# sohmandal/classpose

Measured on AMD Instinct MI355X. Metric: wsi_tiles_per_sec, higher is better.
Workload: dtype bf16; 1 GPU; configs[1]: synthetic 10000x10000 WSI (1936 tiles), tile 256 / overlap 32, conic 7 classes, ViT-L ClassTransformer depth 24 random-init, batch 32 sub-tiles = 8 WSI tiles/step, every step a distinct batch of the rank's shard (tiles sharded k % n_gpus, at most 256 distinct batches resident, longer runs wrap) streamed pinned host -> hipMemcpyAsync inside the timed region (the reader decodes ahead int; slide=10000, tile=256, overlap=32, batch_subtiles=32, distinct_batches=145, records_gathered=2048, decode_ahead_batches_at_t0=4, device_resident_batches_at_t0=1

## Files before the change

classpose_amd/_lib.py:

```python
from __future__ import annotations

import ctypes as C
import os
import subprocess

_HERE = os.path.dirname(os.path.abspath(__file__))
LIB_PATH = os.path.join(_HERE, "libclasspose_hip.so")
DEBUG_LIB_PATH = os.path.join(_HERE, "libclasspose_hip_debug.so")
CSRC = os.path.join(_HERE, "csrc")

ABI_VERSION = 3
DT_BF16, DT_F16, DT_F32 = 0, 1, 2
DTYPE_CODE = {"bf16": DT_BF16, "fp16": DT_F16, "fp32": DT_F32}
PROF_KINDS = ("fc1", "attention", "qkv", "proj", "fc2", "patch_embed", "neck_head")
FC1_KERNEL_NAME = "k_gemm4w<GELU + folded LayerNorm, one wave per SIMD> = void k_gemm4w<1, 0, false>(Gemm4wArgs)"


class CpxTiling(C.Structure):
    _fields_ = [("H", C.c_int), ("W", C.c_int), ("ypad1", C.c_int), ("xpad1", C.c_int),
                ("Ly", C.c_int), ("Lx", C.c_int), ("ny", C.c_int), ("nx", C.c_int),
                ("bsize", C.c_int), ("augment", C.c_int),
                ("ystart", C.c_int * 16), ("xstart", C.c_int * 16)]


# ... 115 lines not shown
    "cpx_head_wgrad_slab_rows": (_i, []),
    "cpx_head_wgrad_workspace_bytes": (_sz, [_i, _i]),
    "cpx_head_wgrad": (_i, [_p, _p, _i, _i, _i, _p, _p, _p, _sz, _p]),
    "cpx_adamw_step": (_i, [_p, _p, _p, _p, C.c_longlong, _d, _d, _d, _d, _d, _d, _d, _p]),
    "cpx_find_contours_ccomp_host": (_i, [_p, _i, _i, _p, _i, _p, _p, _p, _i]),
    "cpx_polygonize_workspace_bytes": (_sz, [_i, _i, _i, _i]),
    "cpx_polygonize_device": (_i, [_p, _p, _p, _i, _i, _i, _i, _d, _p, _p, _i, _p, _p, _p, _p]),
    "cpx_polygonize_host": (_i, [_p, _i, _i, _p, _i, _d, _d, _d, _p, _i, _p]),
    "cpx_dedup_pairs_workspace_bytes": (_sz, [_i, _i, _i]),
    "cpx_dedup_pairs": (_i, [_p, _i, _d, _d, _d, _i, _i, _d, _p, C.c_longlong, _p, _p, _sz, _p]),
    "cpx_write_geojson": (_i, [C.c_char_p, C.c_char_p, _p, C.c_int64, _p, _p, _p, _p, C.c_int64, _p, _i, _d, _d, _i]),
}
_PRIVATE = {
    "cpx_gemm_set_variant": (None, [_i]),
    "cpx_attention_set_variant": (None, [_i]),
    "cpx_gemm_set_nt": (None, [_i]),
    "cpx_follow_set_early_exit": (None, [_i]),
    "cpx_follow_set_lds_window": (None, [_i]),
    "cpx_gemm_set_reverse": (None, [_i]),
    "cpx_attention_set_xcd_order": (None, [_i]),
    "cpx_gemm_set_big": (None, [_i]),
    "cpx_gemm_set_persistent": (None, [_i]),
    "cpx_gemm_set_persistent_qkv": (None, [_i]),
    "cpx_postproc_set_fused": (None, [_i]),
    "cpx_gemm_set_direct": (None, [_i]),
    "cpx_gemm4w": (_i, [_p, _p, _i, _i, _i, _p, _p, _i, _p]),
    "cpx_gemm4w_set_variant": (None, [_i]),
    "cpx_gemm_set_4w": (None, [_i]),
    "cpx_net_set_mlp_parts": (None, [_i]),
    "cpx_gemm_set_balanced": (None, [_i]),
# ... 115 lines not shown
```

classpose_amd/csrc/cpx_attn2w.hip:

```cpp
#include "cpx_internal.h"
#include <type_traits>

namespace {
typedef __attribute__((ext_vector_type(8))) __bf16 bf16x8;
typedef __attribute__((ext_vector_type(8))) _Float16 f16x8;
typedef __attribute__((ext_vector_type(16))) float f32x16;
typedef __attribute__((ext_vector_type(2))) float f32x2;
typedef __attribute__((ext_vector_type(2))) __bf16 bf16x2;
typedef __attribute__((ext_vector_type(2))) _Float16 f16x2;
typedef __attribute__((ext_vector_type(4))) unsigned u32x4;

template <bool F16>
__device__ __forceinline__ f32x16 mfma32(const u32x4 &a, const u32x4 &b, f32x16 c) {
    if constexpr (F16)
        return __builtin_amdgcn_mfma_f32_32x32x16_f16(__builtin_bit_cast(f16x8, a), __builtin_bit_cast(f16x8, b), c, 0, 0, 0);
    else
        return __builtin_amdgcn_mfma_f32_32x32x16_bf16(__builtin_bit_cast(bf16x8, a), __builtin_bit_cast(bf16x8, b), c, 0, 0, 0);
}
template <bool F16>
__device__ __forceinline__ unsigned pack2(float lo, float hi) {
    f32x2 v = {lo, hi};
    if constexpr (F16) return __builtin_bit_cast(unsigned, __builtin_convertvector(v, f16x2));
    else return __builtin_bit_cast(unsigned, __builtin_convertvector(v, bf16x2));
}
__device__ __forceinline__ int pi_perm(int r) { return (r & ~12) | ((r & 4) << 1) | ((r & 8) >> 1); }
template <int OFF>
__device__ __forceinline__ u32x4 a2w_read128(unsigned addr) {
    u32x4 v;
    asm volatile("ds_read_b128 %0, %1 offset:%2" : "=v"(v) : "v"(addr), "n"(OFF));
    return v;
}
}

#define A2W_THREADS 256
#define A2W_SLOT 8192
#define A2W_G_LD 66
#define A2W_LDS_BYTES (4 * A2W_SLOT + 8 * 32 * A2W_G_LD * 2)
static_assert(A2W_LDS_BYTES <= 80 * 1024, "two workgroups per CU");

template <bool F16>
__global__ void __launch_bounds__(A2W_THREADS, 2) k_attention2w(const unsigned short *__restrict__ qkv,
                                                                 const unsigned short *__restrict__ vT,
                                                                 const unsigned short *__restrict__ relh,
                                                                 const unsigned short *__restrict__ relw,
                                                                 unsigned short *__restrict__ out, int xcd_order) {
    extern __shared__ __attribute__((aligned(16))) char a2w_smem[];
    const int tid = threadIdx.x, lane = tid & 63;
    const int wave = __builtin_amdgcn_readfirstlane(tid >> 6);
    const int r = lane & 31, h2 = lane >> 5;
    const int lin = (blockIdx.z * gridDim.y + blockIdx.y) * gridDim.x + blockIdx.x;
    int rg = blockIdx.x, head = blockIdx.y, s = blockIdx.z;
    if (xcd_order) {
        const int j = lin >> 3, pair = (j >> 2) * 8 + (lin & 7);
        rg = j & 3; head = pair & 15; s = pair >> 4;
    }
    const int qh0 = rg * 8 + wave * 2;
    const size_t tok0 = (size_t)s * 1024;
    const int kkey = tid >> 3, vd = tid >> 2;
    const unsigned short *ksrc = qkv + (tok0 + kkey) * 3072 + 1024 + head * 64 + (((tid & 7) ^ ((kkey >> 1) & 7)) * 8);
    const unsigned short *vsrc = vT + (((size_t)s * 16 + head) * 64 + vd) * 1024 + (((tid & 3) ^ ((vd >> 2) & 3)) * 8);
    char *dma_dst = a2w_smem + wave * 1024;
    auto issue = [&](int kh) {
        char *d = dma_dst + (kh & 3) * A2W_SLOT;
        __builtin_amdgcn_global_load_lds((const __attribute__((address_space(1))) void *)(ksrc + (size_t)kh * 32 * 3072),
                                         (__attribute__((address_space(3))) void *)d, 16, 0, 0);
        __builtin_amdgcn_global_load_lds((const __attribute__((address_space(1))) void *)(vsrc + kh * 32),
                                         (__attribute__((address_space(3))) void *)(d + 4096), 16, 0, 0);
    };
    issue(0); issue(1); issue(2);

    u32x4 qf[2][4];
#pragma unroll
    for (int c = 0; c < 2; ++c) {
        const unsigned short *qrow = qkv + (tok0 + (qh0 + c) * 32 + r) * 3072 + head * 64;
#pragma unroll
        for (int ks = 0; ks < 4; ++ks) qf[c][ks] = *reinterpret_cast<const u32x4 *>(qrow + 16 * ks + 8 * h2);
    }
    f32x16 GW[2];
#pragma unroll
    for (int c = 0; c < 2; ++c) {
        _Float16 *G = reinterpret_cast<_Float16 *>(a2w_smem + 4 * A2W_SLOT) + (wave * 2 + c) * 32 * A2W_G_LD;
        auto compute_G = [&](const unsigned short *table) {
// ... 19 lines not shown
    asm volatile("s_waitcnt vmcnt(0) lgkmcnt(0)" ::: "memory");
    __builtin_amdgcn_s_barrier();

    const unsigned lds0 = (unsigned)(size_t)(__attribute__((address_space(3))) char *)a2w_smem;
    const int krow = pi_perm(r);
    unsigned ka[4], va[4];
#pragma unroll
    for (int ks = 0; ks < 4; ++ks) ka[ks] = lds0 + (unsigned)(krow * 128 + (((2 * ks + h2) ^ ((krow >> 1) & 7)) * 16));
#pragma unroll
    for (int db = 0; db < 2; ++db)
#pragma unroll
        for (int st = 0; st < 2; ++st) {
            const int d = db * 32 + r;
            va[db * 2 + st] = lds0 + 4096u + (unsigned)(d * 64 + (((2 * st + h2) ^ ((d >> 2) & 3)) * 16));
        }
    unsigned gaddr[2];
#pragma unroll
    for (int c = 0; c < 2; ++c)
        gaddr[c] = lds0 + 4u * A2W_SLOT + (unsigned)((((wave * 2 + c) * 32 + r) * A2W_G_LD + qh0 + c + 31) * 2);

    u32x4 kf[4], vf[4];
    unsigned ghb[2];
    kf[0] = a2w_read128<0>(ka[0]); kf[1] = a2w_read128<0>(ka[1]);
    kf[2] = a2w_read128<0>(ka[2]); kf[3] = a2w_read128<0>(ka[3]);
    asm volatile("ds_read_u16 %0, %1" : "=v"(ghb[0]) : "v"(gaddr[0]));
    asm volatile("ds_read_u16 %0, %1" : "=v"(ghb[1]) : "v"(gaddr[1]));
    asm volatile("s_waitcnt lgkmcnt(0)" : "+v"(kf[0]), "+v"(kf[1]), "+v"(kf[2]), "+v"(kf[3]), "+v"(ghb[0]), "+v"(ghb[1])::"memory");
    f32x16 S[2], O0[2], O1[2];
    S[0] = mfma32<F16>(kf[0], qf[0][0], GW[0]);
    S[0] = mfma32<F16>(kf[1], qf[0][1], S[0]);
// ... 73 lines not shown
        if constexpr (TAIL == 0) issue(kh + 3);
        unsigned ghn[2] = {0u, 0u};
        if constexpr (TAIL < 3) {
            asm volatile("ds_read_u16 %0, %1" : "=v"(ghn[0]) : "v"(gaddr[0] - 2u * (unsigned)(kh + 1)));
            asm volatile("ds_read_u16 %0, %1" : "=v"(ghn[1]) : "v"(gaddr[1] - 2u * (unsigned)(kh + 1)));
        }
        __builtin_amdgcn_sched_barrier(0);
        qk(C1{});
        if constexpr (!FIRST) pv(C1{});
        softmax(C0{}, ghb[0]);
        __builtin_amdgcn_sched_barrier(0);
        if constexpr (TAIL < 3) {
            kf[0] = a2w_read128<SN * A2W_SLOT>(ka[0]); kf[1] = a2w_read128<SN * A2W_SLOT>(ka[1]);
            kf[2] = a2w_read128<SN * A2W_SLOT>(ka[2]); kf[3] = a2w_read128<SN * A2W_SLOT>(ka[3]);
        }
        vf[0] = a2w_read128<SL * A2W_SLOT>(va[0]); vf[1] = a2w_read128<SL * A2W_SLOT>(va[1]);
        vf[2] = a2w_read128<SL * A2W_SLOT>(va[2]); vf[3] = a2w_read128<SL * A2W_SLOT>(va[3]);
        asm volatile("s_waitcnt lgkmcnt(0)" : "+v"(kf[0]), "+v"(kf[1]), "+v"(kf[2]), "+v"(kf[3]), "+v"(vf[0]), "+v"(vf[1]),
                     "+v"(vf[2]), "+v"(vf[3]), "+v"(ghn[0]), "+v"(ghn[1])::"memory");
        __builtin_amdgcn_sched_barrier(0);
        if constexpr (TAIL < 3) qk(C0{});
        pv(C0{});
        softmax(C1{}, ghb[1]);
        __builtin_amdgcn_sched_barrier(0);
        ghb[0] = ghn[0]; ghb[1] = ghn[1];
    };
    using T0 = integral_constant<int, 0>;
    using NF = std::false_type;
    tile(0, integral_constant<int, 0>{}, integral_constant<int, 1>{}, T0{}, std::true_type{});
    tile(1, integral_constant<int, 1>{}, integral_constant<int, 2>{}, T0{}, NF{});
    tile(2, integral_constant<int, 2>{}, integral_constant<int, 3>{}, T0{}, NF{});
    tile(3, integral_constant<int, 3>{}, integral_constant<int, 0>{}, T0{}, NF{});
// ... 16 lines not shown
        unsigned short *orow = out + (tok0 + (qh0 + c) * 32 + r) * 1024 + head * 64;
#pragma unroll
        for (int db = 0; db < 2; ++db)
#pragma unroll
            for (int g4 = 0; g4 < 4; g4 += 2) {
                const f32x16 &O = db ? O1[c] : O0[c];
                unsigned ax = pack2<F16>(O[4 * g4 + 0] * inv, O[4 * g4 + 1] * inv), ay = pack2<F16>(O[4 * g4 + 2] * inv, O[4 * g4 + 3] * inv);
                unsigned bx = pack2<F16>(O[4 * g4 + 4] * inv, O[4 * g4 + 5] * inv), by = pack2<F16>(O[4 * g4 + 6] * inv, O[4 * g4 + 7] * inv);
                const auto rx = __builtin_amdgcn_permlane32_swap(ax, bx, false, false);
                const auto ry = __builtin_amdgcn_permlane32_swap(ay, by, false, false);
                *reinterpret_cast<uint4 *>(orow + db * 32 + 8 * g4 + 8 * h2) = make_uint4(rx[0], ry[0], rx[1], ry[1]);
            }
    }
}

int cpx_attention2w_launch(int dtype, const void *qkv, const void *vT, const void *rel_h, const void *rel_w,
                           int n_subtiles, void *out, int xcd_order, hipStream_t s) {
    static CpxOncePerDevice once;
    once([] {
        (void)hipFuncSetAttribute((const void *)k_attention2w<true>, hipFuncAttributeMaxDynamicSharedMemorySize, A2W_LDS_BYTES);
        (void)hipFuncSetAttribute((const void *)k_attention2w<false>, hipFuncAttributeMaxDynamicSharedMemorySize, A2W_LDS_BYTES);
    });
    const dim3 grid(4, 16, n_subtiles);
    if (dtype == CPX_DT_F16)
        hipLaunchKernelGGL((k_attention2w<true>), grid, dim3(A2W_THREADS), A2W_LDS_BYTES, s, (const unsigned short *)qkv,
                           (const unsigned short *)vT, (const unsigned short *)rel_h, (const unsigned short *)rel_w,
                           (unsigned short *)out, xcd_order);
    else
        hipLaunchKernelGGL((k_attention2w<false>), grid, dim3(A2W_THREADS), A2W_LDS_BYTES, s, (const unsigned short *)qkv,
                           (const unsigned short *)vT, (const unsigned short *)rel_h, (const unsigned short *)rel_w,
                           (unsigned short *)out, xcd_order);
    CPX_CHECK_LAUNCH();
    return CPX_OK;
}
```

classpose_amd/csrc/cpx_gemm.hip:

```cpp
#include "cpx_internal.h"
#include <type_traits>

typedef __attribute__((ext_vector_type(8))) __bf16 bf16x8;
typedef __attribute__((ext_vector_type(8))) _Float16 f16x8;
typedef __attribute__((ext_vector_type(4))) float f32x4;

#define BM 128
#define BN 128
#define BK 64
#define GEMM_THREADS 256
#define TILE_BYTES (128 * 128)
#define STAGE_BYTES (2 * TILE_BYTES)

template <bool NT_POSSIBLE, bool WT_POSSIBLE = false>
__device__ __forceinline__ void st16(void *p, uint4 v, bool nt, bool wt = false) {
    if (WT_POSSIBLE && wt) {
        typedef unsigned u32x4_t __attribute__((ext_vector_type(4)));
        u32x4_t w = {v.x, v.y, v.z, v.w};
        if (NT_POSSIBLE && nt) asm volatile("global_store_dwordx4 %0, %1, off sc1 nt" ::"v"(p), "v"(w) : "memory");
        else asm volatile("global_store_dwordx4 %0, %1, off sc1" ::"v"(p), "v"(w) : "memory");
    } else if (NT_POSSIBLE && nt) {
        typedef unsigned u32x4_t __attribute__((ext_vector_type(4)));
        u32x4_t w = {v.x, v.y, v.z, v.w};
        __builtin_nontemporal_store(w, reinterpret_cast<u32x4_t *>(p));
// ... 979 lines not shown
                    const int mlh = it * 16 + (tid >> 5);
                    uint4 vv = *reinterpret_cast<const uint4 *>(stg + mlh * G2_EPI_LD + c16 * 16);
                    const int ml = hm * 128 + mlh;
                    const size_t go = (size_t)(m0 + ml) * g.ld_out + n0 + c16 * 8;
                    if constexpr (EPI == CPX_EPI_RESID_BF16) {
                        const uint4 rr = rres[it];
                        unsigned a[4] = {vv.x, vv.y, vv.z, vv.w}, b[4] = {rr.x, rr.y, rr.z, rr.w};
#pragma unroll
                        for (int i = 0; i < 4; ++i) {
                            float lo = from_half<F16>(a[i] & 0xFFFF) + from_half<F16>(b[i] & 0xFFFF);
                            float hi = from_half<F16>(a[i] >> 16) + from_half<F16>(b[i] >> 16);
                            a[i] = pack2<F16>(lo, hi);
                        }
                        vv = make_uint4(a[0], a[1], a[2], a[3]);
                    }
                    if (!DBG || !(g.dbg & 1) || vv.x == 0x12345678u) st16<EPI == CPX_EPI_QKV_BF16, EPI == CPX_EPI_RESID_BF16 || EPI == CPX_EPI_QKV_BF16>((unsigned short *)g.out + go, vv, (g.nt_out & (n0 < 1024 ? 1 : 2)) != 0,
                                                                                        (g.nt_out & (EPI == CPX_EPI_QKV_BF16 ? 16 : 8)) != 0);
                    if constexpr (STATS) {
                        unsigned a[4] = {vv.x, vv.y, vv.z, vv.w};
                        float sm = 0.f, sq = 0.f;
#pragma unroll
                        for (int i = 0; i < 4; ++i) {
                            const float lo = from_half<F16>(a[i] & 0xFFFF), hi = from_half<F16>(a[i] >> 16);
                            sm += lo + hi; sq += lo * lo + hi * hi;
                        }
                        sm = half_wave_sum(sm); sq = half_wave_sum(sq);
                        if (c16 == 16)
                            *reinterpret_cast<float2 *>(g.stats_out + ((size_t)(m0 + ml) * LN_SLOTS + tile_n) * 2) = make_float2(sm, sq);
                    }
                }
                asm volatile("s_waitcnt lgkmcnt(0)" ::: "memory");
                G2_BAR();
// ... 95 lines not shown
                        }
                    }
                    if (f1) launch_gemm256_flags<EPI, F16, F1 | G2F_DBG>(a, s);
                    else launch_gemm256_flags<EPI, F16, G2F_DBG>(a, s);
                    return true;
                }
            }
#endif
            if constexpr (EPI == CPX_EPI_GELU_BF16) {
                if (g_gemm_4w && f1 && a.bias && a.K >= 256 && (a.K / 64) % 2 == 0 &&
                    cpx_gemm4w_gelu_ln(F16 ? 1 : 0, a.A, a.W, a.M, a.N, a.K, a.bias, a.ln_stats, a.ln_colsum, a.out, a.ld_out, s))
                    return true;
            }
            constexpr bool DIRECT_OK = EPI == CPX_EPI_GELU_BF16
#ifdef CPX_DEBUG
                                       || (EPI != CPX_EPI_RESID_BF16 && EPI != CPX_EPI_QKV_BF16)
#endif
                ;
            constexpr bool BAL_OK = EPI == CPX_EPI_RESID_BF16 && !F16;
            const bool bal = BAL_OK && g_gemm_bal != 0 && f1 && a.K >= 256;
            if constexpr (DIRECT_OK) {
                if ((EPI == CPX_EPI_GELU_BF16 ? g_gemm_direct != 0 : g_gemm_direct == 2) && (size_t)a.M * (size_t)a.ld_out * 2 < ((size_t)1 << 31)) {
                    if (f1) launch_gemm256_flags<EPI, F16, F1 | G2F_DIRECT>(a, s);
                    else launch_gemm256_flags<EPI, F16, G2F_DIRECT>(a, s);
                    return true;
                }
            }
            if constexpr (BAL_OK) {
                if (bal) {
                    launch_gemm256_flags<EPI, F16, F1 | G2F_BAL>(a, s);
                    return true;
// ... 56 lines not shown
    if (epilogue == CPX_EPI_F32) return 0;
    if (!g_gemm_big || M % 256 || N % 256 || K < 128) return 0;
    if ((K / 64) % 2 && epilogue != CPX_EPI_POS_BF16) return 0;
    return (M / 256) * (N / 256) >= 256;
}

int cpx_gemm_half(int dtype, const void *A, const void *Wt, int M, int N, int K, int epilogue,
                  const float *bias, const void *aux, void *out, int ld_out,
                  const float *ln_stats, const float *ln_colsum, float *stats_out, void *stream) {
    CPX_REQUIRE(A && Wt && out && (dtype == CPX_DT_BF16 || dtype == CPX_DT_F16));
    const bool f16 = dtype == CPX_DT_F16;
    CPX_REQUIRE(M > 0 && N > 0 && K > 0 && M % BM == 0 && N % BN == 0 && K % BK == 0);
    CPX_REQUIRE(ld_out >= N && ld_out % 4 == 0);
    CPX_REQUIRE((epilogue != CPX_EPI_RESID_BF16 && epilogue != CPX_EPI_POS_BF16 && epilogue != CPX_EPI_QKV_BF16) || aux);
    CPX_REQUIRE(epilogue != CPX_EPI_QKV_BF16 || (N == 3072 && M % 1024 == 0));
    CPX_REQUIRE(!ln_stats || (ln_colsum && epilogue != CPX_EPI_RESID_BF16));
    CPX_REQUIRE(!stats_out || ((epilogue == CPX_EPI_RESID_BF16 || epilogue == CPX_EPI_POS_BF16) && N == 1024 && cpx_gemm_half_uses_big_tile(M, N, K, epilogue)));
    GemmArgs a;
    a.A = (const unsigned short *)A; a.W = (const unsigned short *)Wt;
    a.M = M; a.N = N; a.K = K; a.bias = bias; a.aux = aux; a.out = out; a.ld_out = ld_out;
    a.tiles_n = N / BN; a.n_blocks = (M / BM) * (N / BN);
    a.ln_stats = ln_stats; a.ln_colsum = ln_colsum; a.stats_out = stats_out; a.l2_block = g_gemm_l2; a.dbg = g_gemm_dbg; a.nt_out = g_gemm_nt;
    a.rev_m = (g_gemm_rev && K >= 4096) ? 1 : 0;
    a.conv_c = 0;
    hipStream_t s = (hipStream_t)stream;
    switch (epilogue) {
        case CPX_EPI_BF16: launch_gemm<CPX_EPI_BF16>(a, s, f16); break;
        case CPX_EPI_GELU_BF16: launch_gemm<CPX_EPI_GELU_BF16>(a, s, f16); break;
        case CPX_EPI_RESID_BF16: launch_gemm<CPX_EPI_RESID_BF16>(a, s, f16); break;
        case CPX_EPI_F32: launch_gemm<CPX_EPI_F32>(a, s, f16); break;
        case CPX_EPI_POS_BF16: launch_gemm<CPX_EPI_POS_BF16>(a, s, f16); break;
        case CPX_EPI_RELU_BF16: launch_gemm<CPX_EPI_RELU_BF16>(a, s, f16); break;
        case CPX_EPI_QKV_BF16: launch_gemm<CPX_EPI_QKV_BF16>(a, s, f16); break;
        default: CPX_REQUIRE(!"unknown epilogue");
    }
    CPX_CHECK_LAUNCH();
    return CPX_OK;
}

int cpx_conv3_half(int dtype, const void *x, const void *Wt, int M, int N, int C, int epilogue, const float *bias,
                   void *out, int ld_out, void *stream) {
    CPX_REQUIRE(x && Wt && out && (dtype == CPX_DT_BF16 || dtype == CPX_DT_F16));
    CPX_REQUIRE(M > 0 && M % 1024 == 0 && N > 0 && N % BN == 0 && C > 0 && C % BK == 0);
    CPX_REQUIRE(ld_out >= N && ld_out % 4 == 0 && (epilogue == CPX_EPI_BF16 || epilogue == CPX_EPI_RELU_BF16));
    GemmArgs a;
    a.A = (const unsigned short *)x; a.W = (const unsigned short *)Wt;
    a.M = M; a.N = N; a.K = 9 * C; a.bias = bias; a.aux = nullptr; a.out = out; a.ld_out = ld_out;
    a.tiles_n = N / BN; a.n_blocks = (M / BM) * (N / BN);
// ... 51 lines not shown
```

classpose_amd/csrc/cpx_internal.h:

```cpp
#pragma once
#include "cpx_common.h"
#include <atomic>

struct CpxOncePerDevice {
    std::atomic<unsigned long long> done{0};
    template <class F>
    void operator()(F &&f) {
        int dev = 0;
        (void)hipGetDevice(&dev);
        const unsigned long long bit = 1ull << (dev & 63);
        if (!(done.load(std::memory_order_acquire) & bit)) {
            f();
            done.fetch_or(bit, std::memory_order_release);
        }
    }
};

enum { CPX_PROF_FC1 = 0, CPX_PROF_ATTN = 1, CPX_PROF_QKV = 2, CPX_PROF_PROJ = 3, CPX_PROF_FC2 = 4,
       CPX_PROF_PE = 5,
       CPX_PROF_TAIL = 6,
       CPX_PROF_KINDS = 7 };
struct CpxProf {
    hipEvent_t *ev = nullptr;
    int *kind = nullptr;
// ... 11 lines not shown
    (void)hipEventRecord(p->ev[2 * p->n + 1], s);
    ++p->n;
}

int cpx_gemm_half(int dtype, const void *A, const void *Wt, int M, int N, int K, int epilogue, const float *bias,
                  const void *aux, void *out, int ld_out, const float *ln_stats, const float *ln_colsum,
                  float *stats_out, void *stream);
int cpx_conv3_half(int dtype, const void *x, const void *Wt, int M, int N, int C, int epilogue, const float *bias,
                   void *out, int ld_out, void *stream);
int cpx_row_stats_half(int dtype, const void *x, int rows, float *stats, void *stream);
int cpx_gemm_half_uses_big_tile(int M, int N, int K, int epilogue);
int cpx_gemm4w_gelu_ln(int f16, const void *A, const void *W, int M, int N, int K, const float *bias, const float *ln_stats, const float *ln_colsum,
                       void *out, int ld_out, hipStream_t s);
int cpx_layernorm_half(int dtype, const void *x, const float *w, const float *b, int rows, int C, float eps,
                       void *out, void *stream);
int cpx_attention_half(int dtype, const void *qkv, const void *rel_h, const void *rel_w, int n_subtiles, void *vT_ws,
                       void *out, void *stream, bool transpose_v);
int cpx_attention2w_launch(int dtype, const void *qkv, const void *vT, const void *rel_h, const void *rel_w,
                           int n_subtiles, void *out, int xcd_order, hipStream_t s);

int cpx_gemm_f32(const float *A, const float *Wt, int M, int N, int K, int epilogue, const float *bias,
                 const float *aux, float *out, int ld_out, void *stream);
int cpx_layernorm_f32(const float *x, const float *w, const float *b, int rows, int C, float eps, float *out,
                      void *stream);
int cpx_attention_f32(const float *qkv, const float *rel_h, const float *rel_w, int n_subtiles, float *out,
                      void *stream);
size_t cpx_net_f32_workspace_bytes(int n_subtiles);
size_t cpx_net_f32_neck_offset(int n_subtiles);
int cpx_net_forward_f32(const cpx_net_weights *w, const void *patches, int nS, float *head, void *workspace,
                        size_t workspace_bytes, void *stream);

int cpx_unet_head_run(int dtype, const cpx_conv_op *ops, int n_ops, const void *feat, int nS, float *head, int ld_head,
                      int col0, void *workspace, size_t ws_bytes, void *stream);
size_t cpx_unet_ws_bytes(int dtype, const cpx_conv_op *ops, int n_ops, int nS);
// ... 1 lines not shown
```

classpose_amd/csrc/cpx_net.hip:

```cpp
#include "cpx_internal.h"
#include <algorithm>

typedef __attribute__((ext_vector_type(8))) __bf16 bf16x8;
typedef __attribute__((ext_vector_type(8))) _Float16 f16x8;
typedef __attribute__((ext_vector_type(16))) float f32x16;

template <bool F16>
__device__ __forceinline__ f32x16 mfma32(const uint4 &a, const uint4 &b, f32x16 c) {
    if constexpr (F16)
        return __builtin_amdgcn_mfma_f32_32x32x16_f16(*reinterpret_cast<const f16x8 *>(&a),
                                                      *reinterpret_cast<const f16x8 *>(&b), c, 0, 0, 0);
    else
        return __builtin_amdgcn_mfma_f32_32x32x16_bf16(*reinterpret_cast<const bf16x8 *>(&a),
                                                       *reinterpret_cast<const bf16x8 *>(&b), c, 0, 0, 0);
}
template <bool F16>
__device__ __forceinline__ unsigned short h_from_f32(float f) {
    if constexpr (F16) { _Float16 h = (_Float16)f; return *reinterpret_cast<unsigned short *>(&h); }
    else return f32_to_bf16(f);
}
template <bool F16>
__device__ __forceinline__ float f32_from_h(unsigned short u) {
    if constexpr (F16) return (float)*reinterpret_cast<_Float16 *>(&u);
    else return bf16_to_f32(u);
// ... 293 lines not shown
#pragma unroll
    for (int db = 0; db < 2; ++db)
#pragma unroll
        for (int g4 = 0; g4 < 4; g4 += 2) {
            const f32x16 &O = db ? O1 : O0;
            unsigned ax = pack2<F16>(O[4 * g4 + 0] * inv, O[4 * g4 + 1] * inv), ay = pack2<F16>(O[4 * g4 + 2] * inv, O[4 * g4 + 3] * inv);
            unsigned bx = pack2<F16>(O[4 * g4 + 4] * inv, O[4 * g4 + 5] * inv), by = pack2<F16>(O[4 * g4 + 6] * inv, O[4 * g4 + 7] * inv);
            const auto rx = __builtin_amdgcn_permlane32_swap(ax, bx, false, false);
            const auto ry = __builtin_amdgcn_permlane32_swap(ay, by, false, false);
            *reinterpret_cast<uint4 *>(orow + db * 32 + 8 * g4 + 8 * h2) = make_uint4(rx[0], ry[0], rx[1], ry[1]);
        }
}

CPX_SWITCH(g_att_xcd, 1);
CPX_SWITCH(g_att_v8, 2);
#ifdef CPX_DEBUG
extern "C" void cpx_attention_set_variant(int v8) { g_att_v8 = v8; }
extern "C" void cpx_attention_set_xcd_order(int v) { g_att_xcd = v; }
#endif
extern "C" int cpx_attention_relpos(const void *qkv, const void *rel_h, const void *rel_w,
                                    int n_subtiles, void *vT_ws, void *out, void *stream) {
    return cpx_attention_half(CPX_DT_BF16, qkv, rel_h, rel_w, n_subtiles, vT_ws, out, stream, true);
}
extern "C" int cpx_attention(int dtype, const void *qkv, const void *rel_h, const void *rel_w,
                             int n_subtiles, void *vT_ws, void *out, void *stream) {
    if (dtype == CPX_DT_F32)
        return cpx_attention_f32((const float *)qkv, (const float *)rel_h, (const float *)rel_w, n_subtiles, (float *)out, stream);
    return cpx_attention_half(dtype, qkv, rel_h, rel_w, n_subtiles, vT_ws, out, stream, true);
}
int cpx_attention_half(int dtype, const void *qkv, const void *rel_h, const void *rel_w, int n_subtiles,
                       void *vT_ws, void *out, void *stream, bool transpose_v) {
    CPX_REQUIRE(qkv && rel_h && rel_w && vT_ws && out && n_subtiles > 0);
    CPX_REQUIRE(dtype == CPX_DT_BF16 || dtype == CPX_DT_F16);
#ifdef CPX_DEBUG
    CPX_REQUIRE(g_att_v8 == 2 || g_att_v8 == 7);
#endif
    hipStream_t s = (hipStream_t)stream;
    if (transpose_v)
        hipLaunchKernelGGL(k_v_transpose, dim3(16, 16, n_subtiles), dim3(256), 0, s,
                           (const unsigned short *)qkv, (unsigned short *)vT_ws);
#ifdef CPX_DEBUG
    if (g_att_v8 == 7) {
        const dim3 grid4(8, 16, n_subtiles);
        static CpxOncePerDevice once4;
        once4([] {
            (void)hipFuncSetAttribute((const void *)k_attention4p<true>, hipFuncAttributeMaxDynamicSharedMemorySize, A4_LDS_BYTES);
            (void)hipFuncSetAttribute((const void *)k_attention4p<false>, hipFuncAttributeMaxDynamicSharedMemorySize, A4_LDS_BYTES);
        });
        if (dtype == CPX_DT_F16)
            hipLaunchKernelGGL((k_attention4p<true>), grid4, dim3(ATT_THREADS), A4_LDS_BYTES, s, (const unsigned short *)qkv, (const unsigned short *)vT_ws,
                               (const unsigned short *)rel_h, (const unsigned short *)rel_w, (unsigned short *)out, g_att_xcd);
        else
            hipLaunchKernelGGL((k_attention4p<false>), grid4, dim3(ATT_THREADS), A4_LDS_BYTES, s, (const unsigned short *)qkv, (const unsigned short *)vT_ws,
                               (const unsigned short *)rel_h, (const unsigned short *)rel_w, (unsigned short *)out, g_att_xcd);
        CPX_CHECK_LAUNCH();
        return CPX_OK;
    }
#endif
    return cpx_attention2w_launch(dtype, qkv, vT_ws, rel_h, rel_w, n_subtiles, out, g_att_xcd, s);
}

struct NetWs {
    size_t off_x, off_xn, off_qkv, off_vt, off_ao, off_h, off_neck, off_neck2, off_st, total;
};
static NetWs net_ws(int nS) {
    NetWs w; size_t o = 0; const size_t M = (size_t)nS * 1024;
    auto take = [&](size_t b) { size_t r = o; o = cpx_align_up(o + b, 256); return r; };
    w.off_x = take(M * 1024 * 2);
    w.off_xn = take(M * 1024 * 2);
    w.off_qkv = take(M * 3072 * 2);
    w.off_vt = take(M * 1024 * 2);
    w.off_ao = take(M * 1024 * 2);
    w.off_h = take(M * 4096 * 2);
    w.off_neck = take(M * 256 * 2);
    w.off_neck2 = take(M * 256 * 2);
    w.off_st = take(M * 8 * sizeof(float));
    w.total = o;
    return w;
}
extern "C" size_t cpx_net_workspace_bytes(int n_subtiles, int dtype) {
    if (n_subtiles <= 0) return 0;
    return dtype == CPX_DT_F32 ? cpx_net_f32_workspace_bytes(n_subtiles) : net_ws(n_subtiles).total;
}

extern "C" size_t cpx_net_neck_offset(int n_subtiles, int dtype) {
    if (n_subtiles <= 0 || dtype < CPX_DT_BF16 || dtype > CPX_DT_F32) return 0;
// ... 60 lines not shown
    row0 = pt * 16384;
    rows = pt + 1 < parts ? 16384 : n_subtiles * 1024 - row0;
}

extern "C" int cpx_net_forward(const cpx_net_weights *w, const void *patches, int nS, float *head,
                               void *workspace, size_t workspace_bytes, void *stream) {
    CPX_REQUIRE(w && patches && head && workspace && nS > 0);
    CPX_REQUIRE(w->depth > 0 && w->blocks && w->ld_head % 128 == 0 && w->ld_head >= w->n_head_cols);
    CPX_REQUIRE(w->dtype == CPX_DT_BF16 || w->dtype == CPX_DT_F16 || w->dtype == CPX_DT_F32);
    if (w->dtype == CPX_DT_F32) return cpx_net_forward_f32(w, patches, nS, head, workspace, workspace_bytes, stream);
    NetWs L = net_ws(nS);
    CPX_REQUIRE(workspace_bytes >= L.total);
    const int dt = w->dtype;
    char *ws = (char *)workspace;
    const int M = nS * 1024;
    void *x = ws + L.off_x, *xn = ws + L.off_xn, *qkv = ws + L.off_qkv, *vt = ws + L.off_vt,
         *ao = ws + L.off_ao, *hb = ws + L.off_h, *nk = ws + L.off_neck, *nk2 = ws + L.off_neck2;
    CpxProf *prof = (CpxProf *)w->prof;
    if (prof) prof->phase = (prof->phase + 1) % prof->stride;
    hipStream_t hs = (hipStream_t)stream;
    int rc;
#define RUN(call) do { rc = (call); if (rc) return rc; } while (0)
#define GEMM(A_, W_, N_, K_, EPI_, B_, AUX_, OUT_, LD_) \
    cpx_gemm_half(dt, A_, W_, M, N_, K_, EPI_, B_, AUX_, OUT_, LD_, nullptr, nullptr, nullptr, stream)
#define TIMED(kind_, layer_, call_) do { const bool t_ = cpx_prof_begin(prof, kind_, layer_, hs); RUN(call_); if (t_) cpx_prof_end(prof, hs); } while (0)
    float *st = (float *)(ws + L.off_st);
    const bool fuse = w->fuse_ln != 0;
    const bool big_stats = fuse && cpx_gemm_half_uses_big_tile(M, 1024, 1024, CPX_EPI_RESID_BF16) &&
                           cpx_gemm_half_uses_big_tile(M, 1024, 4096, CPX_EPI_RESID_BF16);
    const bool pe_stats = big_stats && cpx_gemm_half_uses_big_tile(M, 1024, 192, CPX_EPI_POS_BF16);
    TIMED(CPX_PROF_PE, 0, cpx_gemm_half(dt, patches, w->pe_w, M, 1024, 192, CPX_EPI_POS_BF16, w->pe_b, w->pos, x, 1024, nullptr, nullptr,
                                        pe_stats ? st : nullptr, stream));
    if (fuse && !pe_stats) RUN(cpx_row_stats_half(dt, x, M, st, stream));
    for (int i = 0; i < w->depth; ++i) {
        const cpx_block_weights &b = w->blocks[i];
        if (fuse) {
            TIMED(CPX_PROF_QKV, i, cpx_gemm_half(dt, x, b.qkv_w, M, 3072, 1024, CPX_EPI_QKV_BF16, b.qkv_b, vt, qkv, 3072, st, b.qkv_colsum, nullptr, stream));
            TIMED(CPX_PROF_ATTN, i, cpx_attention_half(dt, qkv, b.rel_h, b.rel_w, nS, vt, ao, stream, false));
            TIMED(CPX_PROF_PROJ, i, cpx_gemm_half(dt, ao, b.proj_w, M, 1024, 1024, CPX_EPI_RESID_BF16, b.proj_b, x, x, 1024, nullptr, nullptr, big_stats ? st : nullptr, stream));
            if (!big_stats) RUN(cpx_row_stats_half(dt, x, M, st, stream));
            const int parts = big_stats ? cpx_net_mlp_parts(nS, dt) : 1;
            for (int pt = 0; pt < parts; ++pt) {
                int r0, Mp;
                mlp_part_rows(nS, parts, pt, r0, Mp);
                char *xp = (char *)x + (size_t)r0 * 1024 * 2;
                float *stp = st + (size_t)r0 * 8;
                TIMED(CPX_PROF_FC1, i, cpx_gemm_half(dt, xp, b.fc1_w, Mp, 4096, 1024, CPX_EPI_GELU_BF16, b.fc1_b, nullptr, hb, 4096, stp, b.fc1_colsum, nullptr, stream));
                TIMED(CPX_PROF_FC2, i, cpx_gemm_half(dt, hb, b.fc2_w, Mp, 1024, 4096, CPX_EPI_RESID_BF16, b.fc2_b, xp, xp, 1024, nullptr, nullptr, big_stats ? stp : nullptr, stream));
            }
            if (!big_stats) RUN(cpx_row_stats_half(dt, x, M, st, stream));
            continue;
        }
        RUN(cpx_layernorm_half(dt, x, b.ln1_w, b.ln1_b, M, 1024, 1e-6f, xn, stream));
        TIMED(CPX_PROF_QKV, i, GEMM(xn, b.qkv_w, 3072, 1024, CPX_EPI_QKV_BF16, b.qkv_b, vt, qkv, 3072));
        TIMED(CPX_PROF_ATTN, i, cpx_attention_half(dt, qkv, b.rel_h, b.rel_w, nS, vt, ao, stream, false));
        TIMED(CPX_PROF_PROJ, i, GEMM(ao, b.proj_w, 1024, 1024, CPX_EPI_RESID_BF16, b.proj_b, x, x, 1024));
        RUN(cpx_layernorm_half(dt, x, b.ln2_w, b.ln2_b, M, 1024, 1e-6f, xn, stream));
        TIMED(CPX_PROF_FC1, i, GEMM(xn, b.fc1_w, 4096, 1024, CPX_EPI_GELU_BF16, b.fc1_b, nullptr, hb, 4096));
        TIMED(CPX_PROF_FC2, i, GEMM(hb, b.fc2_w, 1024, 4096, CPX_EPI_RESID_BF16, b.fc2_b, x, x, 1024));
    }
    const bool t_tail = cpx_prof_begin(prof, CPX_PROF_TAIL, 0, hs);
    RUN(GEMM(x, w->neck0_w, 256, 1024, CPX_EPI_BF16, nullptr, nullptr, nk, 256));
    RUN(cpx_layernorm_half(dt, nk, w->neck_ln1_w, w->neck_ln1_b, M, 256, 1e-6f, nk2, stream));
    RUN(cpx_conv3_half(dt, nk2, w->neck2_w, M, 256, 256, CPX_EPI_BF16, nullptr, nk, 256, stream));
    RUN(cpx_layernorm_half(dt, nk, w->neck_ln2_w, w->neck_ln2_b, M, 256, 1e-6f, nk2, stream));
    RUN(GEMM(nk2, w->head_w, w->ld_head, 256, CPX_EPI_F32, w->head_b, nullptr, head, w->ld_head));
    if (w->n_unet_ops > 0) {
        const size_t need = cpx_unet_ws_bytes(dt, w->unet_ops, w->n_unet_ops, nS);
        CPX_REQUIRE(workspace_bytes >= L.total + need);
// ... 189 lines not shown
```

include/classpose_hip_debug.h:

```cpp
#ifndef CLASSPOSE_HIP_DEBUG_H
#define CLASSPOSE_HIP_DEBUG_H
#ifdef __cplusplus
extern "C" {
#endif
void cpx_gemm_set_variant(int glds);
void cpx_gemm_set_big(int on);
void cpx_gemm_set_persistent(int on);
void cpx_gemm_set_persistent_qkv(int on);
void cpx_gemm_set_l2_block(int on);
void cpx_gemm_set_reverse(int on);
void cpx_gemm_set_direct(int mode);
void cpx_gemm_set_balanced(int on);
int cpx_gemm4w(const void *A, const void *W, int M, int N, int K, const float *bias, void *out, int ld_out, void *stream);
void cpx_gemm_set_4w(int on);
void cpx_gemm4w_set_variant(int v);
void cpx_gemm_set_dbg(int mask);
void cpx_net_set_mlp_parts(int on);
void cpx_attention_set_xcd_order(int on);
void cpx_attention_set_variant(int v);
void cpx_postproc_set_fused(int on);
void cpx_gemm_set_nt(int on);
void cpx_follow_set_early_exit(int on);
void cpx_follow_set_lds_window(int on);
int cpx_row_stats_dt(int dtype, const void *x, int rows, float *stats, void *stream);
int cpx_gemm_ln_dt(int dtype, const void *A, const void *Wt, int M, int N, int K, int epilogue,
                   const float *bias, const void *aux, void *out, int ld_out,
                   const float *ln_stats, const float *ln_colsum, float *stats_out, void *stream);
int cpx_im2col3_f32_debug(const float *x, int n_subtiles, float *out, void *stream);
struct cpx_conv_op;
int cpx_unet_head_layout(const struct cpx_conv_op *ops, int n_ops, int n_subtiles, int dtype, size_t *dst_off, int *ld);
#ifdef __cplusplus
}
#endif
#endif
// ... 1 lines not shown
```

Before: 383.6 tiles/s.

## Read V rows directly in attention via LDS transpose reads, drop V transpose output

New measurement: 385.3 tiles/s, median of 6. No clear change (+0.4%).

```diff
diff --git a/classpose_amd/_lib.py b/classpose_amd/_lib.py
--- a/classpose_amd/_lib.py
+++ b/classpose_amd/_lib.py
@@ -153,6 +153,7 @@
 _PRIVATE = {
     "cpx_gemm_set_variant": (None, [_i]),
     "cpx_attention_set_variant": (None, [_i]),
+    "cpx_attention_set_v_rows": (None, [_i]),
     "cpx_gemm_set_nt": (None, [_i]),
     "cpx_follow_set_early_exit": (None, [_i]),
     "cpx_follow_set_lds_window": (None, [_i]),
diff --git a/classpose_amd/csrc/cpx_attn2w.hip b/classpose_amd/csrc/cpx_attn2w.hip
--- a/classpose_amd/csrc/cpx_attn2w.hip
+++ b/classpose_amd/csrc/cpx_attn2w.hip
@@ -9,6 +9,7 @@
 typedef __attribute__((ext_vector_type(2))) __bf16 bf16x2;
 typedef __attribute__((ext_vector_type(2))) _Float16 f16x2;
 typedef __attribute__((ext_vector_type(4))) unsigned u32x4;
+typedef __attribute__((ext_vector_type(2))) unsigned u32x2;
 
 template <bool F16>
 __device__ __forceinline__ f32x16 mfma32(const u32x4 &a, const u32x4 &b, f32x16 c) {
@@ -30,6 +31,13 @@
     asm volatile("ds_read_b128 %0, %1 offset:%2" : "=v"(v) : "v"(addr), "n"(OFF));
     return v;
 }
+template <int OFF>
+__device__ __forceinline__ u32x4 a2w_read_tr(unsigned addr) {
+    u32x2 lo, hi;
+    asm volatile("ds_read_b64_tr_b16 %0, %1 offset:%2" : "=v"(lo) : "v"(addr), "n"(OFF));
+    asm volatile("ds_read_b64_tr_b16 %0, %1 offset:%2" : "=v"(hi) : "v"(addr), "n"(OFF + 512));
+    return (u32x4){lo[0], lo[1], hi[0], hi[1]};
+}
 }
 
 #define A2W_THREADS 256
@@ -38,7 +46,7 @@
 #define A2W_LDS_BYTES (4 * A2W_SLOT + 8 * 32 * A2W_G_LD * 2)
 static_assert(A2W_LDS_BYTES <= 80 * 1024, "two workgroups per CU");
 
-template <bool F16>
+template <bool F16, bool VT>
 __global__ void __launch_bounds__(A2W_THREADS, 2) k_attention2w(const unsigned short *__restrict__ qkv,
                                                                  const unsigned short *__restrict__ vT,
                                                                  const unsigned short *__restrict__ relh,
@@ -59,13 +67,23 @@
     const int kkey = tid >> 3, vd = tid >> 2;
     const unsigned short *ksrc = qkv + (tok0 + kkey) * 3072 + 1024 + head * 64 + (((tid & 7) ^ ((kkey >> 1) & 7)) * 8);
     const unsigned short *vsrc = vT + (((size_t)s * 16 + head) * 64 + vd) * 1024 + (((tid & 3) ^ ((vd >> 2) & 3)) * 8);
+    const unsigned kvoff = (unsigned)(kkey * 3072 + (((tid & 7) ^ ((kkey >> 1) & 7)) * 8)) * 2u;
+    const unsigned vvoff = (unsigned)(kkey * 3072 + (((tid & 7) ^ (((kkey >> 1) & 1) << 2)) * 8)) * 2u;
+    const __amdgpu_buffer_rsrc_t rsrc = __builtin_amdgcn_make_buffer_rsrc((void *)(qkv + tok0 * 3072), 0, 1024 * 3072 * 2, 0x00020000);
+    const unsigned ksoff = (unsigned)(1024 + head * 64) * 2u;
     char *dma_dst = a2w_smem + wave * 1024;
     auto issue = [&](int kh) {
         char *d = dma_dst + (kh & 3) * A2W_SLOT;
-        __builtin_amdgcn_global_load_lds((const __attribute__((address_space(1))) void *)(ksrc + (size_t)kh * 32 * 3072),
-                                         (__attribute__((address_space(3))) void *)d, 16, 0, 0);
-        __builtin_amdgcn_global_load_lds((const __attribute__((address_space(1))) void *)(vsrc + kh * 32),
-                                         (__attribute__((address_space(3))) void *)(d + 4096), 16, 0, 0);
+        if constexpr (VT) {
+            __builtin_amdgcn_global_load_lds((const __attribute__((address_space(1))) void *)(ksrc + (size_t)kh * 32 * 3072),
+                                             (__attribute__((address_space(3))) void *)d, 16, 0, 0);
+            __builtin_amdgcn_global_load_lds((const __attribute__((address_space(1))) void *)(vsrc + kh * 32),
+                                             (__attribute__((address_space(3))) void *)(d + 4096), 16, 0, 0);
+        } else {
+            const unsigned so = ksoff + (unsigned)kh * (32u * 3072u * 2u);
+            __builtin_amdgcn_raw_ptr_buffer_load_lds(rsrc, (__attribute__((address_space(3))) void *)d, 16, kvoff, so, 0, 0);
+            __builtin_amdgcn_raw_ptr_buffer_load_lds(rsrc, (__attribute__((address_space(3))) void *)(d + 4096), 16, vvoff, so + 2048u, 0, 0);
+        }
     };
     issue(0); issue(1); issue(2);
 
@@ -115,6 +133,13 @@
             const int d = db * 32 + r;
             va[db * 2 + st] = lds0 + 4096u + (unsigned)(d * 64 + (((2 * st + h2) ^ ((d >> 2) & 3)) * 16));
         }
+    unsigned vb[2];
+    {
+        const int gi = lane & 15, g1 = (lane >> 4) & 1, q = gi >> 2, p = gi & 3;
+#pragma unroll
+        for (int db = 0; db < 2; ++db)
+            vb[db] = lds0 + 4096u + (unsigned)((8 * h2 + q) * 128 + 16 * ((4 * db + 2 * g1 + (p >> 1)) ^ (((q >> 1) & 1) << 2)) + 8 * (p & 1));
+    }
     unsigned gaddr[2];
 #pragma unroll
     for (int c = 0; c < 2; ++c)
@@ -218,8 +243,13 @@
             kf[0] = a2w_read128<SN * A2W_SLOT>(ka[0]); kf[1] = a2w_read128<SN * A2W_SLOT>(ka[1]);
             kf[2] = a2w_read128<SN * A2W_SLOT>(ka[2]); kf[3] = a2w_read128<SN * A2W_SLOT>(ka[3]);
         }
-        vf[0] = a2w_read128<SL * A2W_SLOT>(va[0]); vf[1] = a2w_read128<SL * A2W_SLOT>(va[1]);
-        vf[2] = a2w_read128<SL * A2W_SLOT>(va[2]); vf[3] = a2w_read128<SL * A2W_SLOT>(va[3]);
+        if constexpr (VT) {
+            vf[0] = a2w_read128<SL * A2W_SLOT>(va[0]); vf[1] = a2w_read128<SL * A2W_SLOT>(va[1]);
+            vf[2] = a2w_read128<SL * A2W_SLOT>(va[2]); vf[3] = a2w_read128<SL * A2W_SLOT>(va[3]);
+        } else {
+            vf[0] = a2w_read_tr<SL * A2W_SLOT>(vb[0]); vf[1] = a2w_read_tr<SL * A2W_SLOT + 2048>(vb[0]);
+            vf[2] = a2w_read_tr<SL * A2W_SLOT>(vb[1]); vf[3] = a2w_read_tr<SL * A2W_SLOT + 2048>(vb[1]);
+        }
         asm volatile("s_waitcnt lgkmcnt(0)" : "+v"(kf[0]), "+v"(kf[1]), "+v"(kf[2]), "+v"(kf[3]), "+v"(vf[0]), "+v"(vf[1]),
                      "+v"(vf[2]), "+v"(vf[3]), "+v"(ghn[0]), "+v"(ghn[1])::"memory");
         __builtin_amdgcn_sched_barrier(0);
@@ -266,22 +296,33 @@
     }
 }
 
-int cpx_attention2w_launch(int dtype, const void *qkv, const void *vT, const void *rel_h, const void *rel_w,
-                           int n_subtiles, void *out, int xcd_order, hipStream_t s) {
+template <bool VT>
+static int attention2w_launch(int dtype, const void *qkv, const void *vT, const void *rel_h, const void *rel_w,
+                              int n_subtiles, void *out, int xcd_order, hipStream_t s) {
     static CpxOncePerDevice once;
     once([] {
-        (void)hipFuncSetAttribute((const void *)k_attention2w<true>, hipFuncAttributeMaxDynamicSharedMemorySize, A2W_LDS_BYTES);
-        (void)hipFuncSetAttribute((const void *)k_attention2w<false>, hipFuncAttributeMaxDynamicSharedMemorySize, A2W_LDS_BYTES);
+        (void)hipFuncSetAttribute((const void *)k_attention2w<true, VT>, hipFuncAttributeMaxDynamicSharedMemorySize, A2W_LDS_BYTES);
+        (void)hipFuncSetAttribute((const void *)k_attention2w<false, VT>, hipFuncAttributeMaxDynamicSharedMemorySize, A2W_LDS_BYTES);
     });
     const dim3 grid(4, 16, n_subtiles);
     if (dtype == CPX_DT_F16)
-        hipLaunchKernelGGL((k_attention2w<true>), grid, dim3(A2W_THREADS), A2W_LDS_BYTES, s, (const unsigned short *)qkv,
+        hipLaunchKernelGGL((k_attention2w<true, VT>), grid, dim3(A2W_THREADS), A2W_LDS_BYTES, s, (const unsigned short *)qkv,
                            (const unsigned short *)vT, (const unsigned short *)rel_h, (const unsigned short *)rel_w,
                            (unsigned short *)out, xcd_order);
     else
-        hipLaunchKernelGGL((k_attention2w<false>), grid, dim3(A2W_THREADS), A2W_LDS_BYTES, s, (const unsigned short *)qkv,
+        hipLaunchKernelGGL((k_attention2w<false, VT>), grid, dim3(A2W_THREADS), A2W_LDS_BYTES, s, (const unsigned short *)qkv,
                            (const unsigned short *)vT, (const unsigned short *)rel_h, (const unsigned short *)rel_w,
                            (unsigned short *)out, xcd_order);
     CPX_CHECK_LAUNCH();
     return CPX_OK;
 }
+int cpx_attention2w_launch(int dtype, const void *qkv, const void *rel_h, const void *rel_w, int n_subtiles, void *out,
+                           int xcd_order, hipStream_t s) {
+    return attention2w_launch<false>(dtype, qkv, nullptr, rel_h, rel_w, n_subtiles, out, xcd_order, s);
+}
+#ifdef CPX_DEBUG
+int cpx_attention2w_vt_launch(int dtype, const void *qkv, const void *vT, const void *rel_h, const void *rel_w,
+                              int n_subtiles, void *out, int xcd_order, hipStream_t s) {
+    return attention2w_launch<true>(dtype, qkv, vT, rel_h, rel_w, n_subtiles, out, xcd_order, s);
+}
+#endif
diff --git a/classpose_amd/csrc/cpx_gemm.hip b/classpose_amd/csrc/cpx_gemm.hip
--- a/classpose_amd/csrc/cpx_gemm.hip
+++ b/classpose_amd/csrc/cpx_gemm.hip
@@ -1017,8 +1017,9 @@
                         }
                         vv = make_uint4(a[0], a[1], a[2], a[3]);
                     }
-                    if (!DBG || !(g.dbg & 1) || vv.x == 0x12345678u) st16<EPI == CPX_EPI_QKV_BF16, EPI == CPX_EPI_RESID_BF16 || EPI == CPX_EPI_QKV_BF16>((unsigned short *)g.out + go, vv, (g.nt_out & (n0 < 1024 ? 1 : 2)) != 0,
-                                                                                        (g.nt_out & (EPI == CPX_EPI_QKV_BF16 ? 16 : 8)) != 0);
+                    constexpr bool QKV = EPI == CPX_EPI_QKV_BF16 || EPI == CPX_EPI_QKV_ROWS;
+                    if (!DBG || !(g.dbg & 1) || vv.x == 0x12345678u) st16<QKV, EPI == CPX_EPI_RESID_BF16 || QKV>((unsigned short *)g.out + go, vv, (g.nt_out & (n0 < 1024 ? 1 : n0 < 2048 ? 2 : 4)) != 0,
+                                                                                        (g.nt_out & (QKV ? 16 : 8)) != 0);
                     if constexpr (STATS) {
                         unsigned a[4] = {vv.x, vv.y, vv.z, vv.w};
                         float sm = 0.f, sq = 0.f;
@@ -1144,7 +1145,7 @@
             }
             constexpr bool DIRECT_OK = EPI == CPX_EPI_GELU_BF16
 #ifdef CPX_DEBUG
-                                       || (EPI != CPX_EPI_RESID_BF16 && EPI != CPX_EPI_QKV_BF16)
+                                       || (EPI != CPX_EPI_RESID_BF16 && EPI != CPX_EPI_QKV_BF16 && EPI != CPX_EPI_QKV_ROWS)
 #endif
                 ;
             constexpr bool BAL_OK = EPI == CPX_EPI_RESID_BF16 && !F16;
@@ -1231,6 +1232,7 @@
     CPX_REQUIRE(ld_out >= N && ld_out % 4 == 0);
     CPX_REQUIRE((epilogue != CPX_EPI_RESID_BF16 && epilogue != CPX_EPI_POS_BF16 && epilogue != CPX_EPI_QKV_BF16) || aux);
     CPX_REQUIRE(epilogue != CPX_EPI_QKV_BF16 || (N == 3072 && M % 1024 == 0));
+    CPX_REQUIRE(epilogue != CPX_EPI_QKV_ROWS || N == 3072);
     CPX_REQUIRE(!ln_stats || (ln_colsum && epilogue != CPX_EPI_RESID_BF16));
     CPX_REQUIRE(!stats_out || ((epilogue == CPX_EPI_RESID_BF16 || epilogue == CPX_EPI_POS_BF16) && N == 1024 && cpx_gemm_half_uses_big_tile(M, N, K, epilogue)));
     GemmArgs a;
@@ -1249,6 +1251,7 @@
         case CPX_EPI_POS_BF16: launch_gemm<CPX_EPI_POS_BF16>(a, s, f16); break;
         case CPX_EPI_RELU_BF16: launch_gemm<CPX_EPI_RELU_BF16>(a, s, f16); break;
         case CPX_EPI_QKV_BF16: launch_gemm<CPX_EPI_QKV_BF16>(a, s, f16); break;
+        case CPX_EPI_QKV_ROWS: launch_gemm<CPX_EPI_QKV_ROWS>(a, s, f16); break;
         default: CPX_REQUIRE(!"unknown epilogue");
     }
     CPX_CHECK_LAUNCH();
diff --git a/classpose_amd/csrc/cpx_internal.h b/classpose_amd/csrc/cpx_internal.h
--- a/classpose_amd/csrc/cpx_internal.h
+++ b/classpose_amd/csrc/cpx_internal.h
@@ -49,10 +49,15 @@
                        void *out, int ld_out, hipStream_t s);
 int cpx_layernorm_half(int dtype, const void *x, const float *w, const float *b, int rows, int C, float eps,
                        void *out, void *stream);
+#define CPX_EPI_QKV_ROWS 7
 int cpx_attention_half(int dtype, const void *qkv, const void *rel_h, const void *rel_w, int n_subtiles, void *vT_ws,
                        void *out, void *stream, bool transpose_v);
-int cpx_attention2w_launch(int dtype, const void *qkv, const void *vT, const void *rel_h, const void *rel_w,
-                           int n_subtiles, void *out, int xcd_order, hipStream_t s);
+int cpx_attention2w_launch(int dtype, const void *qkv, const void *rel_h, const void *rel_w, int n_subtiles, void *out,
+                           int xcd_order, hipStream_t s);
+#ifdef CPX_DEBUG
+int cpx_attention2w_vt_launch(int dtype, const void *qkv, const void *vT, const void *rel_h, const void *rel_w,
+                              int n_subtiles, void *out, int xcd_order, hipStream_t s);
+#endif
 
 int cpx_gemm_f32(const float *A, const float *Wt, int M, int N, int K, int epilogue, const float *bias,
                  const float *aux, float *out, int ld_out, void *stream);
diff --git a/classpose_amd/csrc/cpx_net.hip b/classpose_amd/csrc/cpx_net.hip
--- a/classpose_amd/csrc/cpx_net.hip
+++ b/classpose_amd/csrc/cpx_net.hip
@@ -331,8 +331,10 @@
 
 CPX_SWITCH(g_att_xcd, 1);
 CPX_SWITCH(g_att_v8, 2);
+CPX_SWITCH(g_att_vrows, 1);
 #ifdef CPX_DEBUG
 extern "C" void cpx_attention_set_variant(int v8) { g_att_v8 = v8; }
+extern "C" void cpx_attention_set_v_rows(int on) { g_att_vrows = on; }
 extern "C" void cpx_attention_set_xcd_order(int v) { g_att_xcd = v; }
 #endif
 extern "C" int cpx_attention_relpos(const void *qkv, const void *rel_h, const void *rel_w,
@@ -345,18 +347,20 @@
         return cpx_attention_f32((const float *)qkv, (const float *)rel_h, (const float *)rel_w, n_subtiles, (float *)out, stream);
     return cpx_attention_half(dtype, qkv, rel_h, rel_w, n_subtiles, vT_ws, out, stream, true);
 }
+static bool attention_reads_vt() { return g_att_v8 != 2 || !g_att_vrows; }
 int cpx_attention_half(int dtype, const void *qkv, const void *rel_h, const void *rel_w, int n_subtiles,
                        void *vT_ws, void *out, void *stream, bool transpose_v) {
-    CPX_REQUIRE(qkv && rel_h && rel_w && vT_ws && out && n_subtiles > 0);
+    CPX_REQUIRE(qkv && rel_h && rel_w && out && n_subtiles > 0);
     CPX_REQUIRE(dtype == CPX_DT_BF16 || dtype == CPX_DT_F16);
+    hipStream_t s = (hipStream_t)stream;
 #ifdef CPX_DEBUG
     CPX_REQUIRE(g_att_v8 == 2 || g_att_v8 == 7);
-#endif
-    hipStream_t s = (hipStream_t)stream;
-    if (transpose_v)
-        hipLaunchKernelGGL(k_v_transpose, dim3(16, 16, n_subtiles), dim3(256), 0, s,
-                           (const unsigned short *)qkv, (unsigned short *)vT_ws);
-#ifdef CPX_DEBUG
+    if (attention_reads_vt()) {
+        CPX_REQUIRE(vT_ws);
+        if (transpose_v)
+            hipLaunchKernelGGL(k_v_transpose, dim3(16, 16, n_subtiles), dim3(256), 0, s,
+                               (const unsigned short *)qkv, (unsigned short *)vT_ws);
+    }
     if (g_att_v8 == 7) {
         const dim3 grid4(8, 16, n_subtiles);
         static CpxOncePerDevice once4;
@@ -373,12 +377,13 @@
         CPX_CHECK_LAUNCH();
         return CPX_OK;
     }
+    if (!g_att_vrows) return cpx_attention2w_vt_launch(dtype, qkv, vT_ws, rel_h, rel_w, n_subtiles, out, g_att_xcd, s);
 #endif
-    return cpx_attention2w_launch(dtype, qkv, vT_ws, rel_h, rel_w, n_subtiles, out, g_att_xcd, s);
+    return cpx_attention2w_launch(dtype, qkv, rel_h, rel_w, n_subtiles, out, g_att_xcd, s);
 }
 
 struct NetWs {
-    size_t off_x, off_xn, off_qkv, off_vt, off_ao, off_h, off_neck, off_neck2, off_st, total;
+    size_t off_x, off_xn, off_qkv, off_ao, off_h, off_neck, off_neck2, off_st, total;
 };
 static NetWs net_ws(int nS) {
     NetWs w; size_t o = 0; const size_t M = (size_t)nS * 1024;
@@ -386,7 +391,6 @@
     w.off_x = take(M * 1024 * 2);
     w.off_xn = take(M * 1024 * 2);
     w.off_qkv = take(M * 3072 * 2);
-    w.off_vt = take(M * 1024 * 2);
     w.off_ao = take(M * 1024 * 2);
     w.off_h = take(M * 4096 * 2);
     w.off_neck = take(M * 256 * 2);
@@ -477,8 +481,11 @@
     const int dt = w->dtype;
     char *ws = (char *)workspace;
     const int M = nS * 1024;
-    void *x = ws + L.off_x, *xn = ws + L.off_xn, *qkv = ws + L.off_qkv, *vt = ws + L.off_vt,
+    void *x = ws + L.off_x, *xn = ws + L.off_xn, *qkv = ws + L.off_qkv,
          *ao = ws + L.off_ao, *hb = ws + L.off_h, *nk = ws + L.off_neck, *nk2 = ws + L.off_neck2;
+    void *vt = nullptr;
+    int qkv_epi = CPX_EPI_QKV_ROWS;
+    if (attention_reads_vt()) { vt = hb; qkv_epi = CPX_EPI_QKV_BF16; }
     CpxProf *prof = (CpxProf *)w->prof;
     if (prof) prof->phase = (prof->phase + 1) % prof->stride;
     hipStream_t hs = (hipStream_t)stream;
@@ -498,7 +505,7 @@
     for (int i = 0; i < w->depth; ++i) {
         const cpx_block_weights &b = w->blocks[i];
         if (fuse) {
-            TIMED(CPX_PROF_QKV, i, cpx_gemm_half(dt, x, b.qkv_w, M, 3072, 1024, CPX_EPI_QKV_BF16, b.qkv_b, vt, qkv, 3072, st, b.qkv_colsum, nullptr, stream));
+            TIMED(CPX_PROF_QKV, i, cpx_gemm_half(dt, x, b.qkv_w, M, 3072, 1024, qkv_epi, b.qkv_b, vt, qkv, 3072, st, b.qkv_colsum, nullptr, stream));
             TIMED(CPX_PROF_ATTN, i, cpx_attention_half(dt, qkv, b.rel_h, b.rel_w, nS, vt, ao, stream, false));
             TIMED(CPX_PROF_PROJ, i, cpx_gemm_half(dt, ao, b.proj_w, M, 1024, 1024, CPX_EPI_RESID_BF16, b.proj_b, x, x, 1024, nullptr, nullptr, big_stats ? st : nullptr, stream));
             if (!big_stats) RUN(cpx_row_stats_half(dt, x, M, st, stream));
@@ -515,7 +522,7 @@
             continue;
         }
         RUN(cpx_layernorm_half(dt, x, b.ln1_w, b.ln1_b, M, 1024, 1e-6f, xn, stream));
-        TIMED(CPX_PROF_QKV, i, GEMM(xn, b.qkv_w, 3072, 1024, CPX_EPI_QKV_BF16, b.qkv_b, vt, qkv, 3072));
+        TIMED(CPX_PROF_QKV, i, GEMM(xn, b.qkv_w, 3072, 1024, qkv_epi, b.qkv_b, vt, qkv, 3072));
         TIMED(CPX_PROF_ATTN, i, cpx_attention_half(dt, qkv, b.rel_h, b.rel_w, nS, vt, ao, stream, false));
         TIMED(CPX_PROF_PROJ, i, GEMM(ao, b.proj_w, 1024, 1024, CPX_EPI_RESID_BF16, b.proj_b, x, x, 1024));
         RUN(cpx_layernorm_half(dt, x, b.ln2_w, b.ln2_b, M, 1024, 1e-6f, xn, stream));
diff --git a/include/classpose_hip_debug.h b/include/classpose_hip_debug.h
--- a/include/classpose_hip_debug.h
+++ b/include/classpose_hip_debug.h
@@ -18,6 +18,7 @@
 void cpx_net_set_mlp_parts(int on);
 void cpx_attention_set_xcd_order(int on);
 void cpx_attention_set_variant(int v);
+void cpx_attention_set_v_rows(int on);
 void cpx_postproc_set_fused(int on);
 void cpx_gemm_set_nt(int on);
 void cpx_follow_set_early_exit(int on);
```
